# sstadick/gzp

Measured on AMD Instinct MI355X. Metric: BGZF compress MiB/s at level 1, 550 MiB text, higher is better.
Workload: dtype u8; 1 GPU; Single MI355X: 64 KiB BGZF blocks, level 1, 550 MiB text slab, bit-exact vs libdeflate; slab_bytes=576716800, block_size=65280, blocks=8835, level=1, format=bgzf, parallelism=block-shard x1, device=AMD Radeon Graphics (gfx950:sramecc+:xnack-, 256 CUs)

## Files before the change

### gzp_amd/csrc/gzpx_api.cpp

```cpp
#include <hip/hip_runtime.h>

#include <atomic>
#include <condition_variable>
#include <cmath>
#include <cstdio>
#include <cstdlib>
#include <mutex>
#include <new>
#include <string.h>
#include <vector>

#include "../../include/gzpx.h"
#include "gzpx_device.h"

using namespace gzpx;

namespace {

constexpr size_t kDictSize = 32768;
constexpr uint32_t kMaxBatchBlocks = 16384;
constexpr size_t kMaxScratchBytes = (size_t)24 << 30;

uint32_t multmodp(uint32_t a, uint32_t b) {
    uint32_t m = 1u << 31, p = 0;
// ... 305 lines not shown
                  uint8_t *d_out, size_t out_cap, hipStream_t stream, const SlabResult *prev,
                  SlabResult *result, hipEvent_t dom_b = nullptr, hipEvent_t dom_e = nullptr) {
    const Config &c = ctx->dcfg;
    const Scratch &s = ctx->scratch;
    ProfPairs pp{ctx, ctx->profiling != 0};
    pp.dom_b = dom_b;
    pp.dom_e = dom_e;
    ctx->prof_n = 0;
    auto fork_crc = [&]() -> int {
        HIP_TRY(hipEventRecord(ctx->ev_meta, stream));
        HIP_TRY(hipStreamWaitEvent(ctx->s_side, ctx->ev_meta, 0));
        pp.touch(stream);
        const int tc = pp.begin(6, ctx->s_side);
        launch_crc32(c, d_in, in_len, nb, s, ctx->crc_consts, ctx->s_side);
        pp.end(tc, ctx->s_side);
        HIP_TRY(hipEventRecord(ctx->ev_crc, ctx->s_side));
        return GZPX_OK;
    };
    const uint32_t fork_sel = (c.debug >> 8) & 3u;
    const uint32_t fork_at = fork_sel == 0 ? (c.level <= 1 ? 1u : 0u) : fork_sel == 1 ? 0u : fork_sel == 2 ? 2u : 1u;
    int t = pp.begin(c.level == 0 ? 0 : 1, stream);
    launch_candidates(c, d_in, in_len, nb, is_last, s, stream);
    pp.end(t, stream);
    if (fork_at == 1) {
        const int rc = fork_crc();
        if (rc != GZPX_OK) return rc;
    }
    if (c.level <= 1) {
        t = pp.begin(2, stream);
        launch_match(c, d_in, in_len, nb, s, stream);
        pp.end(t, stream);
        if (fork_at == 2) {
            const int rc = fork_crc();
            if (rc != GZPX_OK) return rc;
        }
        t = pp.begin(3, stream);
        launch_parse(c, d_in, in_len, nb, s, stream);
        pp.end(t, stream);
    } else {
        t = pp.begin(2, stream);
        if (c.level >= 10) {
            launch_near_optimal(c, d_in, nb, s, stream);
        } else if (c.lazy) {
            launch_lazy(c, d_in, nb, s, stream);
        } else {
            launch_hc(c, d_in, nb, s, stream);
        }
        pp.end(t, stream);
    }
    if (fork_at == 0 || (fork_at == 2 && c.level > 1)) {
        const int rc = fork_crc();
        if (rc != GZPX_OK) return rc;
    }
    t = pp.begin(4, stream);
    launch_hist(c, nb, s, stream);
    pp.end(t, stream);
    t = pp.begin(5, stream);
    launch_huffman(c, nb, s, stream);
    pp.end(t, stream);
    t = pp.begin(7, stream);
    launch_scan(nb, s, prev, result, stream);
    pp.end(t, stream);
    HIP_TRY(hipStreamWaitEvent(stream, ctx->ev_crc, 0));
    pp.touch(stream);
    t = pp.begin(8, stream);
    launch_emit(c, d_in, in_len, nb, s, d_out, out_cap, stream);
    pp.end(t, stream);
    HIP_TRY(hipGetLastError());
    if (pp.on && !dom_b) {
        HIP_TRY(hipStreamSynchronize(stream));
        for (int i = 0; i < ctx->prof_n; i++) {
            float ms = 0;
            HIP_TRY(hipEventElapsedTime(&ms, ctx->prof_ev[ctx->prof_b[i]], ctx->prof_ev[ctx->prof_e[i]]));
            ctx->stage_ms[ctx->prof_stage[i]] += ms;
        }
    }
    ctx->last_nb = nb;
    return GZPX_OK;
}

int enqueue_snap_batch(gzpx_ctx *ctx, const uint8_t *d_in, size_t in_len, uint32_t nb, uint8_t *d_out,
                       size_t out_cap, hipStream_t stream, const SlabResult *prev, SlabResult *result,
                       hipEvent_t dom_b = nullptr, hipEvent_t dom_e = nullptr) {
    const Scratch &s = ctx->scratch;
    const uint32_t bs = (uint32_t)ctx->cfg.buffer_size;
    ProfPairs pp{ctx, ctx->profiling != 0};
    pp.dom_b = dom_b;
    pp.dom_e = dom_e;
    ctx->prof_n = 0;
    if (ctx->snap.dbg)
        HIP_TRY(hipMemsetAsync(ctx->snap.dbg, 0,
                               (size_t)nb * snap_chunks_per_buffer(bs) * 8 * sizeof(uint64_t), stream));
    int t = pp.begin(2, stream);
    launch_snap_chunk(d_in, in_len, bs, nb, ctx->snap, stream);
    pp.end(t, stream);
    t = pp.begin(7, stream);
    launch_snap_frame(in_len, bs, nb, s, ctx->snap, stream);
    launch_scan(nb, s, prev, result, stream);
    pp.end(t, stream);
    t = pp.begin(8, stream);
    launch_snap_emit(d_in, in_len, bs, nb, s, ctx->snap, d_out, out_cap, stream);
    pp.end(t, stream);
    HIP_TRY(hipGetLastError());
    if (pp.on && !dom_b) {
        HIP_TRY(hipStreamSynchronize(stream));
        for (int i = 0; i < ctx->prof_n; i++) {
            float ms = 0;
            HIP_TRY(hipEventElapsedTime(&ms, ctx->prof_ev[ctx->prof_b[i]], ctx->prof_ev[ctx->prof_e[i]]));
            ctx->stage_ms[ctx->prof_stage[i]] += ms;
// ... 2121 lines not shown
```

### gzp_amd/csrc/gzpx_device.h

```cpp
#pragma once
#include <stdint.h>

namespace gzpx {

constexpr unsigned kTile = 65536;
constexpr unsigned kMaxBlockSize = 1u << 26;
constexpr unsigned kSeqPerSub = 8192;
constexpr unsigned kSoftMaxSub = 65535;
constexpr unsigned kMinBlockLen = 5000;
constexpr unsigned kNumLitlen = 288;
constexpr unsigned kNumOffset = 32;
constexpr unsigned kHistStride = kNumLitlen + kNumOffset;
constexpr unsigned kHdrWords = 160;
constexpr unsigned kCodeWords = kNumLitlen + kNumOffset;

constexpr uint32_t kTokMatch = 0x80000000u;

enum SubType : uint32_t { kStored = 0, kStatic = 1, kDynamic = 2 };

enum BlockStatus : uint32_t {
    kStatusOk = 0,
    kStatusBlockSizeExceeded = 2,
    kStatusInternal = 3,
};
// ... 69 lines not shown
    uint8_t *len8;
    uint32_t *which;
    uint16_t *alt;
    uint16_t *d4;
    uint8_t *lz_len;
    uint16_t *lz_dist;
    HcState *hc;
    uint32_t *pending;
    uint32_t *tok;
    uint32_t *redo;
    uint32_t *claim;
    uint32_t *hist;
    uint32_t *codes;
    uint32_t *hdr;
    uint64_t *out_off;
    uint32_t *sizes;
    uint32_t no_lanes;
    void *no_state;
    uint8_t *no_cache;
    uint8_t *no_nodes;
};

constexpr uint32_t kSnapStageBytes = 76544;
struct SnapScratch {
    uint8_t *stage;
    uint32_t *clen;
    uint32_t *crc;
    uint32_t *coff;
    uint64_t *dbg;
};
inline uint32_t snap_chunks_per_buffer(uint32_t bs) { return (bs + 65535u) / 65536u; }
void launch_snap_chunk(const uint8_t *slab, uint64_t slab_len, uint32_t bs, uint32_t nb, const SnapScratch &ss,
                       hipStream_t stream);
void launch_snap_frame(uint64_t slab_len, uint32_t bs, uint32_t nb, const Scratch &s, const SnapScratch &ss,
                       hipStream_t stream);
void launch_snap_emit(const uint8_t *slab, uint64_t slab_len, uint32_t bs, uint32_t nb, const Scratch &s,
                      const SnapScratch &ss, uint8_t *out, uint64_t out_cap, hipStream_t stream);

void launch_init_meta(const Config &cfg, uint64_t slab_len, uint32_t nb, int is_last,
                      const Scratch &s, hipStream_t stream);
void launch_candidates(const Config &cfg, const uint8_t *slab, uint64_t slab_len, uint32_t nb, int is_last,
                       const Scratch &s, hipStream_t stream);
void launch_match(const Config &cfg, const uint8_t *slab, uint64_t slab_len, uint32_t nb,
                  const Scratch &s, hipStream_t stream);
void launch_parse(const Config &cfg, const uint8_t *slab, uint64_t slab_len, uint32_t nb,
                  const Scratch &s, hipStream_t stream);
void launch_hc(const Config &cfg, const uint8_t *slab, uint32_t nb, const Scratch &s, hipStream_t stream);
void launch_lazy(const Config &cfg, const uint8_t *slab, uint32_t nb, const Scratch &s, hipStream_t stream);
size_t no_lane_bytes();
size_t no_cache_bytes();
size_t no_nodes_bytes(uint32_t block_size);
void launch_near_optimal_tables(void *lanes, uint32_t n_lanes, const uint8_t *d_tables, hipStream_t stream);
void launch_near_optimal(const Config &cfg, const uint8_t *slab, uint32_t nb, const Scratch &s, hipStream_t stream);
void launch_hist(const Config &cfg, uint32_t nb, const Scratch &s, hipStream_t stream);
void launch_huffman(const Config &cfg, uint32_t nb, const Scratch &s, hipStream_t stream);
void launch_crc32(const Config &cfg, const uint8_t *slab, uint64_t slab_len, uint32_t nb,
                  const Scratch &s, const CrcConsts &cc, hipStream_t stream);
void launch_scan(uint32_t nb, const Scratch &s, const SlabResult *prev, SlabResult *result, hipStream_t stream);
void launch_emit(const Config &cfg, const uint8_t *slab, uint64_t slab_len, uint32_t nb,
                 const Scratch &s, uint8_t *out, uint64_t out_cap, hipStream_t stream);

struct DBlockHost {
    uint64_t in_off;
    uint32_t size, isize, crc, status, produced, nmatch;
    uint32_t cyc[8];
};
struct InflateScratch {
    void *mlist = nullptr;
    uint32_t *tfirst = nullptr;
    uint32_t *redo = nullptr;
    uint32_t *summary = nullptr;
    int n_cu = 0;
    int big_members = 0;
};
enum { kInflateRouteSeg = 0, kInflateRouteWave = 1 };
size_t inflate_mlist_bytes(uint64_t out_cap, uint64_t nb);
size_t inflate_tfirst_bytes(uint64_t out_cap, uint64_t nb);
void launch_inflate(uint32_t hdr_len, const uint8_t *d_in, const uint64_t *d_offsets, const uint32_t *d_sizes,
                    uint32_t nb, void *d_blk, uint64_t *d_out_off, uint8_t *d_out, uint64_t out_cap,
                    uint32_t *d_crc_found, const CrcConsts &cc, int debug, hipEvent_t ev_begin,
                    hipEvent_t ev_end, hipStream_t stream, const InflateScratch &sc, int route, hipEvent_t ev_mid = nullptr);

struct MemberScanScratch {
    uint32_t *seg_count = nullptr;
    uint32_t *seg_off = nullptr;
    uint64_t *pos = nullptr;
    uint32_t *size = nullptr;
    uint32_t *succ = nullptr;
    uint32_t *jump[2] = {nullptr, nullptr};
    uint32_t *idx = nullptr;
    uint32_t *rec = nullptr;
    uint32_t cap = 0;
};
void launch_member_scan(int format, const uint8_t *d_in, uint64_t in_len, uint32_t seg_bytes, uint32_t n_seg,
                        uint32_t rounds, const MemberScanScratch &m, hipStream_t stream);
void launch_member_emit(const MemberScanScratch &m, uint32_t n_emit, uint64_t *d_offsets, uint32_t *d_sizes,
                        hipStream_t stream);
void launch_member_index(const uint8_t *d_in, const uint64_t *d_offsets, const uint32_t *d_sizes, uint32_t nb, void *d_blk,
                         uint64_t *d_out_off, hipStream_t stream);

struct RrIndex {
    const uint64_t *off;
    const uint32_t *size;
    const uint64_t *ustart;
    uint32_t n;
};
// ... 21 lines not shown
```

### gzp_amd/csrc/gzpx_kernels.hip

```cpp
#include <hip/hip_runtime.h>
#include <type_traits>
#include <cstring>

#include "gzpx_device.h"

#ifdef GZPX_EXPERIMENT
#define GZPX_EXP(cfg, bit) (((cfg).debug >> (bit)) & 1u)
#else
#define GZPX_EXP(cfg, bit) 0u
#endif

namespace gzpx {


__device__ __forceinline__ void wave_sync() {
    __builtin_amdgcn_fence(__ATOMIC_SEQ_CST, "wavefront");
    __builtin_amdgcn_wave_barrier();
    __builtin_amdgcn_fence(__ATOMIC_SEQ_CST, "wavefront");
}

__device__ __forceinline__ uint32_t rdlane(uint32_t v, uint32_t l) {
    return (uint32_t)__builtin_amdgcn_readlane((int)v, (int)l);
}
__device__ __forceinline__ uint32_t uniform(uint32_t v) { return (uint32_t)__builtin_amdgcn_readfirstlane((int)v); }

#if defined(__HIP_DEVICE_COMPILE__)
#define GZPX_PIN_VGPR(x) asm volatile("" : "+v"(x))
#else
#define GZPX_PIN_VGPR(x) ((void)0)
#endif

__device__ __forceinline__ uint32_t lz_hash15(uint32_t v) { return (v * 0x1E35A7BDu) >> 17; }

__device__ __forceinline__ uint32_t load_le32_global(const uint8_t *p) {
    const uintptr_t a = (uintptr_t)p;
    const uint32_t *w = (const uint32_t *)(a & ~(uintptr_t)3);
    return __builtin_amdgcn_alignbyte(w[1], w[0], (uint32_t)(a & 3));
}

__device__ __forceinline__ uint32_t wave_reduce_add(uint32_t v) {
    for (int m = 32; m >= 1; m >>= 1) v += __shfl_xor(v, m);
    return v;
}

__device__ __forceinline__ uint32_t wave_inclusive_scan(uint32_t v, unsigned lane) {
    for (int d = 1; d < 64; d <<= 1) {
        uint32_t t = __shfl_up(v, d);
        if (lane >= (unsigned)d) v += t;
    }
    return v;
}

template <int CTRL, int ROW_MASK>
__device__ __forceinline__ uint32_t dpp_zero(uint32_t v) {
// ... 2791 lines not shown
        }
        __syncthreads();
    }
}

struct HuffLds {
    union {
        uint32_t key[kNumLitlen];
        uint32_t nfreq[kNumLitlen];
        uint32_t hdr[kHdrWords];
    };
    union {
        uint32_t sfreq[kNumLitlen];
        struct {
            uint32_t sfreq_low[32];
            uint16_t items[kNumLitlen + kNumOffset];
        };
    };
    union {
        uint32_t freq[kNumLitlen];
        struct {
            uint32_t freq_low[kNumLitlen / 2];
            uint16_t parent[kNumLitlen];
        };
    };
    uint32_t lcw[kNumLitlen];
    uint16_t ssym[kNumLitlen];
    uint8_t depth[kNumLitlen];
    uint8_t lens[kNumLitlen + kNumOffset];
    uint8_t olens[kNumOffset + 2];
    uint8_t plens[32];
    uint32_t ocw[kNumOffset];
    uint32_t pcw[32];
    uint32_t pfreq[32];
    uint32_t len_counts[16];
    uint32_t misc[8];
};
static_assert(sizeof(HuffLds) <= 6400, "HuffLds: 25 workgroups per CU");
static_assert(kHdrWords <= kNumLitlen, "header bits fit region A");


__device__ __forceinline__ uint32_t reg5_get(const uint32_t (&r)[5], uint32_t k) {
    const uint32_t j = k >> 6, l = k & 63u;
    uint32_t v = rdlane(r[0], l);
    const uint32_t v1 = rdlane(r[1], l), v2 = rdlane(r[2], l), v3 = rdlane(r[3], l), v4 = rdlane(r[4], l);
    v = j == 1 ? v1 : v;
    v = j == 2 ? v2 : v;
    v = j == 3 ? v3 : v;
    v = j == 4 ? v4 : v;
    return v;
}

template <uint32_t NCH, uint32_t MAXL>
__device__ void make_code(HuffLds &h, uint32_t num_syms, uint32_t compat, uint8_t *lens, uint32_t *cw, uint32_t lane) {
    constexpr uint32_t max_len = MAXL;
    uint32_t used = 0;
    for (uint32_t base = 0; base < num_syms; base += 64) {
        const uint32_t s = base + lane;
        uint32_t f = 0;
        if (s < num_syms) {
            f = h.freq[s];
            h.key[s] = f ? ((f << 10) | s) : 0xFFFFFFFFu;
            lens[s] = 0;
            cw[s] = 0;
        }
        used += (uint32_t)__popcll(__ballot(f != 0));
    }
    wave_sync();
    if (used < 2) {
        if (used == 0 && compat == 1) return;
        if (lane == 0) {
            uint32_t sym = 0;
            if (used)
                for (uint32_t s = 0; s < num_syms; s++)
                    if (h.freq[s]) sym = s;
            const uint32_t other = sym ? sym : 1;
            lens[0] = 1;
            cw[0] = 0;
            lens[other] = 1;
            cw[other] = 1;
        }
        wave_sync();
        return;
    }
    {
        uint32_t at = 0;
        uint32_t k0 = lane < num_syms ? h.key[lane] : 0xFFFFFFFFu;
        for (uint32_t base = 0; base < num_syms; base += 64) {
            const uint32_t s1 = base + 64 + lane;
            const uint32_t k1 = s1 < num_syms ? h.key[s1] : 0xFFFFFFFFu;
            wave_sync();
            const bool u = k0 != 0xFFFFFFFFu;
            const unsigned long long m = __ballot(u);
            if (u) h.key[at + (uint32_t)__popcll(m & ((1ull << lane) - 1ull))] = k0;
            at += (uint32_t)__popcll(m);
            k0 = k1;
        }
    }
    wave_sync();
    for (uint32_t base = 0; base < used; base += 64) {
        const uint32_t s = base + lane;
        const uint32_t k = s < used ? h.key[s] : 0u;
        uint32_t rank = 0;
        for (uint32_t j = 0; j < used; j++) rank += h.key[j] < k ? 1u : 0u;
        if (s < used) {
            h.sfreq[rank] = k >> 10;
            h.ssym[rank] = (uint16_t)(k & 1023u);
// ... 82 lines not shown
                h.len_counts[l]--;
                h.len_counts[l + 1] += 2;
            }
        }
    }
    wave_sync();
    for (uint32_t base = 0; base < used; base += 64) {
        const uint32_t k = base + lane;
        if (k < used) {
            uint32_t acc = 0, l = max_len;
            for (; l >= 1; l--) {
                acc += h.len_counts[l];
                if (k < acc) break;
            }
            lens[h.ssym[k]] = (uint8_t)l;
        }
    }
    wave_sync();
    uint32_t next_code[16];
    next_code[0] = 0;
    next_code[1] = 0;
#pragma unroll
    for (uint32_t l = 2; l <= MAXL; l++) next_code[l] = (next_code[l - 1] + h.len_counts[l - 1]) << 1;
    const uint64_t lane_below = (1ull << lane) - 1ull;
    for (uint32_t base = 0; base < num_syms; base += 64) {
        const uint32_t s = base + lane;
        const uint32_t myl = s < num_syms ? lens[s] : 0;
        uint32_t code = 0;
#pragma unroll
        for (uint32_t l = 1; l <= MAXL; l++) {
            const uint64_t m = __ballot(myl == l);
            if (myl == l) code = next_code[l] + (uint32_t)__popcll(m & lane_below);
            next_code[l] += (uint32_t)__popcll(m);
        }
        if (myl) cw[s] = __brev(code) >> (32 - myl);
    }
    wave_sync();
}

__device__ __forceinline__ void hdr_or_bits(uint32_t *hdr, uint32_t bitpos, uint32_t v, uint32_t nbits) {
    const uint32_t w = bitpos >> 5, sh = bitpos & 31u;
    atomicOr(&hdr[w], v << sh);
    if (sh + nbits > 32) atomicOr(&hdr[w + 1], v >> (32 - sh));
}

__device__ __forceinline__ void hdr_put(uint32_t *hdr, uint32_t &bitpos, uint32_t v, uint32_t nbits) {
    if (!nbits) return;
    const uint32_t w = bitpos >> 5, sh = bitpos & 31u;
    hdr[w] |= v << sh;
    if (sh + nbits > 32) hdr[w + 1] |= v >> (32 - sh);
    bitpos += nbits;
}

#ifndef GZPX_HUFF_WAVES
#define GZPX_HUFF_WAVES 6
#endif
__global__ __launch_bounds__(64, GZPX_HUFF_WAVES) void k_huffman(Config cfg, BlockMeta *__restrict__ meta_all,
                                                SubMeta *__restrict__ sub_all,
                                                const uint32_t *__restrict__ hist_all,
                                                uint32_t *__restrict__ codes_all,
                                                uint32_t *__restrict__ hdr_all) {
    __shared__ HuffLds h;
    const uint32_t lane = threadIdx.x;
    const uint32_t b = blockIdx.x;
    BlockMeta *meta = meta_all + b;
    SubMeta *sub = sub_all + (uint64_t)b * cfg.max_sub;
    const uint32_t n = meta->n;
    const uint32_t hdr_len = hdr_len_of(cfg.format);
    const uint32_t eof_len = (meta->is_last && cfg.format == 0) ? 28u : 0u;

    if (n <= cfg.passthrough) {
        if (lane == 0) {
            const uint32_t chunks = n ? (n + 65534u) / 65535u : 1u;
            const uint32_t c = 5u * chunks + n;
            meta->nsub = 1;
            meta->ntok = 0;
            sub[0].type = kStored;
            sub[0].tok_begin = 0;
            sub[0].tok_end = 0;
            sub[0].byte_begin = 0;
            sub[0].byte_len = n;
            sub[0].bit_begin = 0;
            sub[0].hdr_bits = 0;
            sub[0].is_final = 1;
            meta->payload_bytes = c;
            meta->framed_bytes = hdr_len + c + 8 + eof_len;
            if (cfg.format == 0 && c >= 65536u) meta->status = kStatusBlockSizeExceeded;
        }
        return;
    }

    const uint32_t nsub = meta->nsub;
    uint32_t bitpos = 0;
    for (uint32_t s = 0; s < nsub; s++) {
        const uint32_t *hist = hist_all + ((uint64_t)b * cfg.max_sub + s) * kHistStride;
        uint32_t *codes = codes_all + ((uint64_t)b * cfg.max_sub + s) * kCodeWords;
        uint32_t *hdr_out = hdr_all + ((uint64_t)b * cfg.max_sub + s) * kHdrWords;
        const uint32_t block_length = sub[s].byte_len;
        const uint32_t is_final = sub[s].is_final;

#ifdef GZPX_EXPERIMENT
        unsigned long long hx_t = __builtin_readcyclecounter();
#define GZPX_HLAP(slot)                                                                               \
    do {                                                                                              \
        const unsigned long long t_ = __builtin_readcyclecounter();                                   \
        if (lane == 0) atomicAdd(&g_exp_huff[(b & 1023u) * 8u + (slot)], t_ - hx_t);                  \
        hx_t = t_;                                                                                    \
    } while (0)
#else
#define GZPX_HLAP(slot) ((void)0)
#endif
        uint32_t lfreq[5];
        for (uint32_t k = 0; k < 5; k++) {
            const uint32_t i = lane + 64 * k;
            lfreq[k] = i < kNumLitlen ? hist[i] + (i == 256 ? 1u : 0u) : 0;
            if (i < kNumLitlen) h.freq[i] = lfreq[k];
        }
        wave_sync();
        GZPX_HLAP(0);
        make_code<5, 14>(h, kNumLitlen, cfg.compat, h.lens, h.lcw, lane);
        GZPX_HLAP(1);
        const uint32_t ofreq = lane < kNumOffset ? hist[kNumLitlen + lane] : 0;
        if (lane < kNumOffset) h.freq[lane] = ofreq;
        wave_sync();
        make_code<1, 15>(h, kNumOffset, cfg.compat, h.olens, h.ocw, lane);
        GZPX_HLAP(2);
        wave_sync();

        uint32_t num_litlen, num_offset;
        {
            uint32_t hi_l = 0;
            for (uint32_t k = 0; k < 5; k++) {
                const uint32_t i = lane + 64 * k;
                if (i < kNumLitlen && h.lens[i]) hi_l = i + 1;
            }
            for (int m = 32; m >= 1; m >>= 1) {
                const uint32_t o = __shfl_xor(hi_l, m);
                hi_l = o > hi_l ? o : hi_l;
            }
            num_litlen = hi_l < 257 ? 257 : hi_l;
            uint32_t hi_o = (lane < kNumOffset && h.olens[lane]) ? lane + 1 : 0;
            for (int m = 32; m >= 1; m >>= 1) {
                const uint32_t o = __shfl_xor(hi_o, m);
                hi_o = o > hi_o ? o : hi_o;
            }
            num_offset = hi_o < 1 ? 1 : hi_o;
        }
        if (lane < num_offset) h.lens[num_litlen + lane] = h.olens[lane];
        if (lane < 32) h.pfreq[lane] = 0;
        wave_sync();
        uint32_t num_items;
        {
            const uint32_t num_lens = num_litlen + num_offset;
            uint32_t lr[5];
            unsigned long long sm[5];
#pragma unroll
            for (uint32_t k = 0; k < 5; k++) {
                const uint32_t idx = lane + 64 * k;
                lr[k] = idx < num_lens ? (uint32_t)h.lens[idx] : 0xFFu;
            }
#pragma unroll
            for (uint32_t k = 0; k < 5; k++) {
                uint32_t prev = (uint32_t)__shfl_up((int)lr[k], 1);
                const uint32_t carry = k ? rdlane(lr[k ? k - 1 : 0], 63) : 0x100u;
                if (lane == 0) prev = carry;
                sm[k] = __ballot(lr[k] != prev);
            }
            uint32_t ni = 0;
#pragma unroll
            for (uint32_t k = 0; k < 5; k++) {
                if (64 * k >= num_lens) break;
                uint32_t before = 0, after = num_lens;
#pragma unroll
                for (uint32_t j = 0; j < 5; j++)
                    if (j < k && sm[j]) before = 64 * j + 63u - (uint32_t)__clzll((long long)sm[j]);
// ... 413 lines not shown
    uint64_t inc = mine;
    for (int d = 1; d < 64; d <<= 1) {
        const uint64_t t = __shfl_up(inc, d);
        if (lane >= (unsigned)d) inc += t;
    }
    if (lane == 63) wsum[wave] = inc;
    __syncthreads();
    uint64_t run = prev ? prev->total : 0;
    uint64_t total = run;
    for (uint32_t w = 0; w < kScanThreads / 64; w++) {
        const uint64_t v = wsum[w];
        if (w < wave) run += v;
        total += v;
    }
    run += inc - mine;
#pragma unroll 8
    for (uint32_t i = i0; i < i1; i++) {
        const uint32_t v = meta[i].framed_bytes;
        sizes[i] = v;
        out_off[i] = run;
        run += v;
    }
    if (tid == 0) {
        const uint32_t f = fail_s;
        out_off[nb] = total;
        result->total = total;
        result->fail_block = f;
        result->fail_status = f != 0xFFFFFFFFu ? meta[f].status : kStatusOk;
    }
}

constexpr uint32_t kStageWords = 18432;

__device__ __forceinline__ void stage_or_bits(uint32_t *stage, uint32_t bitpos, uint64_t v) {
    const uint32_t w = bitpos >> 5, sh = bitpos & 31u;
    const uint64_t t = v << sh;
    const uint32_t x0 = (uint32_t)t, x1 = (uint32_t)(t >> 32);
    const uint32_t x2 = sh ? (uint32_t)(v >> (64 - sh)) : 0u;
    if (x0) atomicOr(&stage[w], x0);
    if (x1) atomicOr(&stage[w + 1], x1);
    if (x2) atomicOr(&stage[w + 2], x2);
}

__device__ __forceinline__ void stage_put_byte(uint32_t *stage, uint32_t byte_idx, uint32_t v) {
    atomicOr(&stage[byte_idx >> 2], (v & 0xFFu) << (8u * (byte_idx & 3u)));
}

constexpr uint32_t kEmitThreads = 1024;

__device__ __forceinline__ void stage_flush(const uint32_t *stage, uint8_t *dst_aligned,
                                            uint32_t win_base, uint32_t upto, uint32_t lead,
                                            uint32_t end_byte, uint32_t tid) {
    const uint32_t words = (upto - win_base + 3) >> 2;
    for (uint32_t w = tid; w < words; w += kEmitThreads) {
        const uint32_t v = stage[w];
        const uint32_t b0 = win_base + 4 * w;
        if (b0 >= lead && b0 + 4 <= end_byte && b0 + 4 <= upto) {
            *(uint32_t *)(dst_aligned + b0) = v;
        } else {
            for (uint32_t k = 0; k < 4; k++)
                if (b0 + k >= lead && b0 + k < end_byte && b0 + k < upto)
                    dst_aligned[b0 + k] = (uint8_t)(v >> (8 * k));
        }
    }
}

__device__ __forceinline__ void emit_block(const Config &cfg, const uint8_t *__restrict__ slab,
                                           const BlockMeta *__restrict__ meta_all,
                                           const SubMeta *__restrict__ sub_all,
                                           const uint32_t *__restrict__ tok_all,
                                           const uint32_t *__restrict__ codes_all,
                                           const uint32_t *__restrict__ hdr_all,
                                           const uint64_t *__restrict__ out_off,
                                           uint8_t *__restrict__ out, uint64_t out_cap, const uint32_t b,
                                           uint32_t *stage, uint32_t *codes, uint32_t *wsum, const uint8_t *lslot) {
    const uint32_t tid = threadIdx.x;
    const BlockMeta *meta = meta_all + b;
    const SubMeta *sub = sub_all + (uint64_t)b * cfg.max_sub;
    const uint32_t n = meta->n;
    const uint32_t framed = meta->framed_bytes;
    const uint32_t c = meta->payload_bytes;
    const uint64_t dst_off = out_off[b];
    if (meta->status != kStatusOk || dst_off + framed > out_cap) return;
    const uint8_t *in = slab + (uint64_t)b * cfg.block_size;
    const uint32_t hdr_len = hdr_len_of(cfg.format);
    const uint32_t lead = (uint32_t)(((uintptr_t)out + dst_off) & 3u);
    uint8_t *dst_aligned = out + dst_off - lead;
    const uint32_t end_byte = lead + framed;
    uint32_t win_base = 0;

    for (uint32_t i = tid; i < kStageWords; i += kEmitThreads) stage[i] = 0;
    __syncthreads();

    if (tid == 0) {
        const uint32_t hb = lead;
        stage_put_byte(stage, hb + 0, 0x1f);
        stage_put_byte(stage, hb + 1, 0x8b);
        stage_put_byte(stage, hb + 2, 8);
        stage_put_byte(stage, hb + 3, 4);
        stage_put_byte(stage, hb + 8, cfg.xfl);
        stage_put_byte(stage, hb + 9, 255);
        if (cfg.format == 0) {
            const uint32_t bsize = c + 25;
            stage_put_byte(stage, hb + 10, 6);
            stage_put_byte(stage, hb + 12, 'B');
            stage_put_byte(stage, hb + 13, 'C');
            stage_put_byte(stage, hb + 14, 2);
            stage_put_byte(stage, hb + 16, bsize);
            stage_put_byte(stage, hb + 17, bsize >> 8);
        } else {
            const uint32_t tot = c + 28;
            stage_put_byte(stage, hb + 10, 8);
            stage_put_byte(stage, hb + 12, 'I');
            stage_put_byte(stage, hb + 13, 'G');
            stage_put_byte(stage, hb + 14, 4);
            stage_put_byte(stage, hb + 16, tot);
            stage_put_byte(stage, hb + 17, tot >> 8);
            stage_put_byte(stage, hb + 18, tot >> 16);
            stage_put_byte(stage, hb + 19, tot >> 24);
        }
    }

    const uint32_t *tok = tok_all + (uint64_t)b * cfg.stride;
    const uint32_t nsub = meta->nsub;
    uint32_t bitpos = 8u * (lead + hdr_len);
    auto ensure = [&](uint32_t need_bits) {
        if (((bitpos + need_bits + 7) >> 3) + 16u <= 4u * kStageWords) return;
        __syncthreads();
        const uint32_t upto_rel = (bitpos >> 3) & ~3u;
        stage_flush(stage, dst_aligned, win_base, win_base + upto_rel, lead, end_byte, tid);
        const uint32_t keep = stage[upto_rel >> 2];
        __syncthreads();
        for (uint32_t i = tid; i < kStageWords; i += kEmitThreads) stage[i] = 0;
        __syncthreads();
        if (tid == 0) stage[0] = keep;
        win_base += upto_rel;
        bitpos -= 8u * upto_rel;
        __syncthreads();
    };
    for (uint32_t s = 0; s < nsub; s++) {
        const SubMeta sm = sub[s];
        if (sm.type == kStored) {
            uint32_t left = sm.byte_len, src = sm.byte_begin;
            do {
                const uint32_t chunk = left > 65535u ? 65535u : left;
                const bool last_chunk = chunk == left;
                ensure(64);
                if (tid == 0) stage_or_bits(stage, bitpos, (sm.is_final && last_chunk) ? 1u : 0u);
                bitpos = (bitpos + 3 + 7u) & ~7u;
                if (tid == 0) {
                    const uint32_t bytepos = bitpos >> 3;
                    stage_put_byte(stage, bytepos + 0, chunk);
                    stage_put_byte(stage, bytepos + 1, chunk >> 8);
                    stage_put_byte(stage, bytepos + 2, ~chunk);
                    stage_put_byte(stage, bytepos + 3, (~chunk) >> 8);
                }
                bitpos += 32;
                for (uint32_t done = 0; done < chunk; done += 16384u) {
                    const uint32_t piece = chunk - done < 16384u ? chunk - done : 16384u;
                    ensure(8u * piece);
                    const uint32_t bytepos = bitpos >> 3;
                    for (uint32_t i = tid; i < piece; i += kEmitThreads)
                        stage_put_byte(stage, bytepos + i, in[src + done + i]);
                    bitpos += 8u * piece;
                }
                src += chunk;
                left -= chunk;
            } while (left);
            __syncthreads();
            continue;
        }
        __syncthreads();
        const uint32_t *cd = codes_all + ((uint64_t)b * cfg.max_sub + s) * kCodeWords;
        for (uint32_t i = tid; i < kCodeWords; i += kEmitThreads) codes[i] = cd[i];
        const uint32_t *hw = hdr_all + ((uint64_t)b * cfg.max_sub + s) * kHdrWords;
        const uint32_t nhw = (sm.hdr_bits + 31) >> 5;
        ensure(32u * kHdrWords);
        for (uint32_t i = tid; i < nhw; i += kEmitThreads) stage_or_bits(stage, bitpos + 32 * i, hw[i]);
        bitpos += sm.hdr_bits;
        __syncthreads();
        const uint32_t tok_last = meta->ntok - 1;
        uint32_t tnext[4];
#pragma unroll
        for (uint32_t j = 0; j < 4; j++) {
            const uint32_t i = sm.tok_begin + 4 * tid + j;
            tnext[j] = tok[i < tok_last ? i : tok_last];
        }
        for (uint32_t tb = sm.tok_begin; tb < sm.tok_end; tb += 4 * kEmitThreads) {
            ensure(4u * kEmitThreads * 48u);
            const uint32_t t0 = tb + 4 * tid;
            uint64_t bits[4];
            uint32_t nbits[4], sum = 0;
            uint32_t tcur[4];
#pragma unroll
            for (uint32_t j = 0; j < 4; j++) tcur[j] = tnext[j];
#pragma unroll
            for (uint32_t j = 0; j < 4; j++) {
                const uint32_t i = t0 + 4 * kEmitThreads + j;
                tnext[j] = tok[i < tok_last ? i : tok_last];
            }
#pragma unroll
            for (uint32_t j = 0; j < 4; j++) {
                bits[j] = 0;
                nbits[j] = 0;
                if (t0 + j < sm.tok_end) {
                    const uint32_t t = tcur[j];
                    if (t & kTokMatch) {
                        const uint32_t len = t & 0x1FFu, off = (t >> 9) & 0xFFFFu;
                        uint32_t os, oe, ov;
                        const uint32_t lt = lslot[len - 3u];
                        const uint32_t ls = lt & 31u, le = lt >> 5, lv = (len - 3u) & ((1u << le) - 1u);
                        offset_slot(off, os, oe, ov);
                        const uint32_t lc = codes[257 + ls], oc = codes[kNumLitlen + os];
                        const uint32_t lpart = (lc & 0xFFFFu) | (lv << (lc >> 16)), lbits = (lc >> 16) + le;
                        const uint32_t opart = (oc & 0xFFFFu) | (ov << (oc >> 16)), obits = (oc >> 16) + oe;
                        bits[j] = (uint64_t)lpart | ((uint64_t)opart << lbits);
                        nbits[j] = lbits + obits;
                    } else {
                        const uint32_t lc = codes[t];
                        bits[j] = lc & 0xFFFFu;
                        nbits[j] = lc >> 16;
                    }
                    sum += nbits[j];
                }
            }
            uint32_t total;
            const uint32_t ex = block_exclusive_scan<kEmitThreads / 64>(sum, wsum, &total);
            uint32_t off_bits = bitpos + ex, accn = 0;
            uint64_t acc = 0;
#pragma unroll
            for (uint32_t j = 0; j < 4; j++) {
                if (accn + nbits[j] > 64) {
                    stage_or_bits(stage, off_bits, acc);
                    off_bits += accn;
                    acc = 0;
                    accn = 0;
                }
                acc |= bits[j] << accn;
                accn += nbits[j];
            }
            if (accn) stage_or_bits(stage, off_bits, acc);
            bitpos += total;
        }
        ensure(64);
        if (tid == 0) {
            const uint32_t ec = codes[256];
            stage_or_bits(stage, bitpos, ec & 0xFFFFu);
        }
        bitpos += codes[256] >> 16;
        __syncthreads();
    }

    ensure(8u * (8u + 28u + 8u));
    if (tid == 0) {
        const uint32_t fb = lead + hdr_len + c - win_base;
        const uint32_t crc = meta->crc;
        for (uint32_t k = 0; k < 4; k++) {
            stage_put_byte(stage, fb + k, crc >> (8 * k));
            stage_put_byte(stage, fb + 4 + k, n >> (8 * k));
        }
        if (meta->is_last && cfg.format == 0) {
            const uint8_t eof[28] = {0x1f, 0x8b, 0x08, 0x04, 0, 0, 0, 0, 0x00, 0xff, 0x06, 0x00, 0x42, 0x43,
                                     0x02, 0x00, 0x1b, 0x00, 0x03, 0x00, 0, 0, 0, 0, 0, 0, 0, 0};
            for (uint32_t k = 0; k < 28; k++) stage_put_byte(stage, fb + 8 + k, eof[k]);
        }
    }
    __syncthreads();
    stage_flush(stage, dst_aligned, win_base, end_byte, lead, end_byte, tid);
}

__global__ __launch_bounds__(kEmitThreads, 8) void k_emit(Config cfg, const uint8_t *__restrict__ slab,
                                              const BlockMeta *__restrict__ meta_all,
                                              const SubMeta *__restrict__ sub_all,
                                              const uint32_t *__restrict__ tok_all,
                                              const uint32_t *__restrict__ codes_all,
                                              const uint32_t *__restrict__ hdr_all,
                                              const uint64_t *__restrict__ out_off,
                                              uint8_t *__restrict__ out, uint64_t out_cap, uint32_t nb) {
    __shared__ uint32_t stage[kStageWords];
    __shared__ uint32_t codes[kCodeWords];
    __shared__ uint32_t wsum[kEmitThreads / 64];
    __shared__ uint8_t lslot[256];
    if (threadIdx.x < 256) {
        uint32_t ls, le, lv;
        length_slot(threadIdx.x + 3, ls, le, lv);
        lslot[threadIdx.x] = (uint8_t)(ls | (le << 5));
    }
    for (uint32_t b = blockIdx.x; b < nb; b += gridDim.x) {
        __syncthreads();
        emit_block(cfg, slab, meta_all, sub_all, tok_all, codes_all, hdr_all, out_off, out, out_cap, b, stage, codes, wsum,
                   lslot);
    }
}

template <bool GWIN>
struct InfLdsT {
    uint32_t win[GWIN ? 1 : 8192];
    uint32_t lfast[1024];
    uint32_t ofast[256];
    uint32_t inr[256];
    uint32_t own[64];
    uint16_t lsorted[288];
    uint16_t osorted[32];
    uint8_t lens[320];
    uint32_t lcount[16], lfirst[16], loffs[16];
    uint32_t ocount[16], ofirst[16], ooffs[16];
};

#ifndef GZPX_INF_R
#define GZPX_INF_R 2
#endif
constexpr uint32_t kInfR = GZPX_INF_R;

enum InflateStatus : uint32_t { kInfOk = 0, kInfBadData = 1, kInfInsufficientSpace = 2, kInfShortOutput = 3 };

enum InfKind { kInfLitlen = 0, kInfOffset = 1, kInfPrecode = 2 };

template <int KIND>
__device__ __forceinline__ uint32_t inflate_entry(uint32_t sym, uint32_t cl) {
    if (KIND == kInfPrecode) return cl | (sym << 8);
    if (KIND == kInfLitlen) {
        if (sym < 256) return cl | (sym << 8);
        if (sym == 256) return cl | (2u << 4);
        const uint32_t slot = sym - 257;
        uint32_t base, xb = 0;
        if (slot < 8) {
            base = 3 + slot;
        } else if (slot >= 28) {
            base = 258;
        } else {
            xb = (slot - 4) >> 2;
            base = 3 + ((4 + (slot & 3)) << xb);
        }
        return cl | (1u << 4) | (xb << 8) | (base << 16);
    }
    if (sym > 29) return cl | (1u << 4);
    uint32_t base, xb = 0;
    if (sym < 4) {
        base = 1 + sym;
    } else {
        xb = (sym - 2) >> 1;
        base = 1 + ((2 + (sym & 1)) << xb);
    }
    return cl | (xb << 8) | (base << 16);
// ... 838 lines not shown
        hipLaunchKernelGGL(k_match_hc, dim3(nb), dim3(1024), 0, stream, cfg, slab, (const BlockMeta *)s.meta, s.hc,
                           (const uint16_t *)s.cand, (const uint16_t *)s.d4, s.len8, s.which, s.alt,
                           (uint8_t *)nullptr, (uint16_t *)nullptr);
    };
    auto parse_round = [&](uint32_t may_list_stale) {
        hipLaunchKernelGGL(k_parse_hc<false>, dim3(nb), dim3(kMpThreads), 0, stream, cfg, slab, s.meta, s.sub, s.hc,
                           (const uint8_t *)s.len8, (const uint32_t *)s.which, (const uint16_t *)s.alt, s.tok,
                           s.pending, s.redo, may_list_stale);
    };
    const bool sparse = !(cfg.debug & 16u) && (cfg.level >= 3 || (cfg.debug & 32u));
    if (sparse)
        hipLaunchKernelGGL(k_match_hc_sparse, dim3(nb), dim3(1024), 0, stream, cfg, slab, (const BlockMeta *)s.meta, s.hc,
                           (const uint16_t *)s.cand, (const uint16_t *)s.d4, s.len8, s.which, s.alt);
    else
        dense();
    hipLaunchKernelGGL(k_hc_orphan, dim3(nb), dim3(64), 0, stream, cfg, slab, (const BlockMeta *)s.meta, s.hc,
                       (const uint16_t *)s.cand, (const uint16_t *)s.d4, s.len8, s.which, s.alt, (uint8_t *)nullptr,
                       (uint16_t *)nullptr);
    parse_round(1u);
    if (sparse) {
        const uint32_t wgs = cfg.n_cu ? cfg.n_cu : 256u;
        hipLaunchKernelGGL(k_match_hc_stale, dim3(wgs), dim3(1024), 0, stream, cfg, slab, (const BlockMeta *)s.meta,
                           s.hc, (const uint16_t *)s.cand, (const uint16_t *)s.d4, s.len8, s.which, s.alt,
                           (const uint32_t *)s.redo);
    }
    parse_round(0u);
    hipLaunchKernelGGL(k_parse_hc<true>, dim3(nb), dim3(kMpThreads), 0, stream, cfg, slab, s.meta, s.sub, s.hc,
                       (const uint8_t *)s.len8, (const uint32_t *)s.which, (const uint16_t *)s.alt, s.tok,
                       s.pending, s.redo, 0u);
}

void launch_lazy(const Config &cfg, const uint8_t *slab, uint32_t nb, const Scratch &s, hipStream_t stream) {
    hipLaunchKernelGGL(k_hc_init, dim3((nb + 255) / 256), dim3(256), 0, stream, nb, s.hc, s.pending);
    hipLaunchKernelGGL(k_match_hc, dim3(nb), dim3(1024), 0, stream, cfg, slab, (const BlockMeta *)s.meta, s.hc,
                       (const uint16_t *)s.cand, (const uint16_t *)s.d4, s.len8, s.which, s.alt, s.lz_len,
                       s.lz_dist);
    hipLaunchKernelGGL(k_hc_orphan, dim3(nb), dim3(64), 0, stream, cfg, slab, (const BlockMeta *)s.meta, s.hc,
                       (const uint16_t *)s.cand, (const uint16_t *)s.d4, s.len8, s.which, s.alt, s.lz_len, s.lz_dist);
    if (cfg.lazy >= 2)
        hipLaunchKernelGGL(k_parse_lazy<3>, dim3(nb), dim3(64), 0, stream, cfg, slab, s.meta, s.sub,
                           (const uint8_t *)s.len8, (const uint16_t *)s.alt, (const uint8_t *)s.lz_len,
                           (const uint16_t *)s.lz_dist, s.tok);
    else
        hipLaunchKernelGGL(k_parse_lazy<2>, dim3(nb), dim3(64), 0, stream, cfg, slab, s.meta, s.sub,
                           (const uint8_t *)s.len8, (const uint16_t *)s.alt, (const uint8_t *)s.lz_len,
                           (const uint16_t *)s.lz_dist, s.tok);
}

void launch_hist(const Config &cfg, uint32_t nb, const Scratch &s, hipStream_t stream) {
    hipLaunchKernelGGL(k_hist, dim3(nb), dim3(256), 0, stream, cfg, (const BlockMeta *)s.meta,
                       (const SubMeta *)s.sub, (const uint32_t *)s.tok, s.hist);
}

void launch_huffman(const Config &cfg, uint32_t nb, const Scratch &s, hipStream_t stream) {
    hipLaunchKernelGGL(k_huffman, dim3(nb), dim3(64), 0, stream, cfg, s.meta, s.sub,
                       (const uint32_t *)s.hist, s.codes, s.hdr);
}

void launch_crc32(const Config &cfg, const uint8_t *slab, uint64_t, uint32_t nb, const Scratch &s,
                  const CrcConsts &cc, hipStream_t stream) {
    hipLaunchKernelGGL(k_crc32, dim3(nb), dim3(kCrcSmall), 0, stream, cfg, slab, s.meta, cc);
}

void launch_scan(uint32_t nb, const Scratch &s, const SlabResult *prev, SlabResult *result, hipStream_t stream) {
    hipLaunchKernelGGL(k_scan, dim3(1), dim3(kScanThreads), 0, stream, nb, (const BlockMeta *)s.meta,
                       s.out_off, s.sizes, prev, result);
}

void launch_emit(const Config &cfg, const uint8_t *slab, uint64_t, uint32_t nb, const Scratch &s,
                 uint8_t *out, uint64_t out_cap, hipStream_t stream) {
    hipLaunchKernelGGL(k_emit, dim3(nb), dim3(kEmitThreads), 0, stream, cfg, slab, (const BlockMeta *)s.meta,
                       (const SubMeta *)s.sub, (const uint32_t *)s.tok, (const uint32_t *)s.codes,
                       (const uint32_t *)s.hdr, (const uint64_t *)s.out_off, out, out_cap, nb);
}

void launch_inflate(uint32_t hdr_len, const uint8_t *d_in, const uint64_t *d_offsets, const uint32_t *d_sizes,
                    uint32_t nb, void *d_blk, uint64_t *d_out_off, uint8_t *d_out, uint64_t out_cap,
                    uint32_t *d_crc_found, const CrcConsts &cc, int debug, hipEvent_t ev_begin,
                    hipEvent_t ev_end, hipStream_t stream, const InflateScratch &sc, int route, hipEvent_t ev_mid) {
    DBlock *blk = (DBlock *)d_blk;
    const bool seg = route != kInflateRouteWave && sc.mlist && sc.tfirst && sc.redo;
    hipLaunchKernelGGL(k_dinit, dim3((nb + 255) / 256), dim3(256), 0, stream, nb, d_in, d_offsets, d_sizes, blk,
                       seg ? sc.redo : (uint32_t *)nullptr);
    hipLaunchKernelGGL(k_dscan, dim3(1), dim3(256), 0, stream, nb, (const DBlock *)blk, d_out_off);
    if (ev_begin) (void)hipEventRecord(ev_begin, stream);
    if (seg) {
        LzMatch *ml = (LzMatch *)sc.mlist;
        const bool big = sc.big_members != 0;
        const uint32_t seg_wgs = (uint32_t)(sc.n_cu > 0 ? sc.n_cu : 256) * 4u * GZPX_SEG_WAVES / (big ? (uint32_t)kSegBigW : (uint32_t)kSegSmallW);
        const uint32_t seg_grid = nb < seg_wgs ? nb : seg_wgs;
        uint32_t *seg_hint = sc.summary ? sc.summary + 15 : nullptr;
#define GZPX_LAUNCH_SEG(DBG_)                                                                                              \
    do {                                                                                                                   \
        if (big)                                                                                                           \
            hipLaunchKernelGGL((k_inflate_seg<DBG_, kSegBigW>), dim3(seg_grid), dim3(64 * kSegBigW), 0, stream, hdr_len,   \
                               d_in, blk, (const uint64_t *)d_out_off, d_out, out_cap, ml, sc.tfirst, sc.redo, nb, seg_hint); \
        else                                                                                                               \
            hipLaunchKernelGGL((k_inflate_seg<DBG_, kSegSmallW>), dim3(seg_grid), dim3(64 * kSegSmallW), 0, stream, hdr_len, d_in, blk, \
                               (const uint64_t *)d_out_off, d_out, out_cap, ml, sc.tfirst, sc.redo, nb, seg_hint);         \
        if (ev_mid) (void)hipEventRecord(ev_mid, stream);                                                                  \
    } while (0)
        if (debug == 1) {
            GZPX_LAUNCH_SEG(true);
            hipLaunchKernelGGL((k_lzcopy<false>), dim3(nb), dim3(kLcThreads), 0, stream, blk, (const uint64_t *)d_out_off,
                               d_out, (const LzMatch *)ml, (const uint32_t *)sc.tfirst, sc.redo, d_crc_found, cc);
            hipLaunchKernelGGL((k_inflate<true, true>), dim3(nb), dim3(64), 0, stream, hdr_len, d_in, blk,
                               (const uint64_t *)d_out_off, d_out, out_cap, (const uint32_t *)sc.redo);
        } else if (debug == 2) {
            GZPX_LAUNCH_SEG(false);
// ... 91 lines not shown
```

Baseline: 159,700 MiB/s.

## Fold symbol histogram into the Huffman kernel and skip separate hist launch

When the block size fits in one tile, the Huffman kernel now tallies literal/length and offset frequencies itself from the token stream. It uses LDS atomics over four padded copies and a length-slot lookup table, so the separate histogram kernel launch and its global hist buffer round trip are dropped. The tally runs with a single 64-lane wave per block instead of the 256-thread hist kernel, which trades launch and global-memory traffic for a longer serial phase inside the Huffman kernel. The tally lives in a union overlaid on the existing LDS struct, so occupancy is meant to stay the same.

```diff
diff --git a/gzp_amd/csrc/gzpx_api.cpp b/gzp_amd/csrc/gzpx_api.cpp
--- a/gzp_amd/csrc/gzpx_api.cpp
+++ b/gzp_amd/csrc/gzpx_api.cpp
@@ -381,9 +381,11 @@
         const int rc = fork_crc();
         if (rc != GZPX_OK) return rc;
     }
-    t = pp.begin(4, stream);
-    launch_hist(c, nb, s, stream);
-    pp.end(t, stream);
+    if (!huffman_tallies(c)) {
+        t = pp.begin(4, stream);
+        launch_hist(c, nb, s, stream);
+        pp.end(t, stream);
+    }
     t = pp.begin(5, stream);
     launch_huffman(c, nb, s, stream);
     pp.end(t, stream);
diff --git a/gzp_amd/csrc/gzpx_device.h b/gzp_amd/csrc/gzpx_device.h
--- a/gzp_amd/csrc/gzpx_device.h
+++ b/gzp_amd/csrc/gzpx_device.h
@@ -145,6 +145,7 @@
 size_t no_nodes_bytes(uint32_t block_size);
 void launch_near_optimal_tables(void *lanes, uint32_t n_lanes, const uint8_t *d_tables, hipStream_t stream);
 void launch_near_optimal(const Config &cfg, const uint8_t *slab, uint32_t nb, const Scratch &s, hipStream_t stream);
+bool huffman_tallies(const Config &cfg);
 void launch_hist(const Config &cfg, uint32_t nb, const Scratch &s, hipStream_t stream);
 void launch_huffman(const Config &cfg, uint32_t nb, const Scratch &s, hipStream_t stream);
 void launch_crc32(const Config &cfg, const uint8_t *slab, uint64_t slab_len, uint32_t nb,
diff --git a/gzp_amd/csrc/gzpx_kernels.hip b/gzp_amd/csrc/gzpx_kernels.hip
--- a/gzp_amd/csrc/gzpx_kernels.hip
+++ b/gzp_amd/csrc/gzpx_kernels.hip
@@ -1,5 +1,6 @@
 #include <hip/hip_runtime.h>
 #include <type_traits>
+#include <cstddef>
 #include <cstring>
 
 #include "gzpx_device.h"
@@ -2897,7 +2898,7 @@
 }
 
 template <uint32_t NCH, uint32_t MAXL>
-__device__ void make_code(HuffLds &h, uint32_t num_syms, uint32_t compat, uint8_t *lens, uint32_t *cw, uint32_t lane) {
+__device__ __forceinline__ void make_code(HuffLds &h, uint32_t num_syms, uint32_t compat, uint8_t *lens, uint32_t *cw, uint32_t lane) {
     constexpr uint32_t max_len = MAXL;
     uint32_t used = 0;
     for (uint32_t base = 0; base < num_syms; base += 64) {
@@ -3086,15 +3087,75 @@
     bitpos += nbits;
 }
 
+constexpr uint32_t kTallyCopies = 4;
+constexpr uint32_t kTallyLitPad = kNumLitlen + 1;
+constexpr uint32_t kTallyOffPad = kNumOffset + 1;
+constexpr uint32_t kTallyOffAt = kTallyCopies * kTallyLitPad;
+constexpr uint32_t kTallyWords = kTallyOffAt + kTallyCopies * kTallyOffPad;
+union HuffShared {
+    HuffLds h;
+    struct {
+        uint32_t tally[kTallyWords];
+        uint8_t lslot[512];
+    };
+};
+static_assert(sizeof(HuffShared) == sizeof(HuffLds), "the tally lives inside HuffLds: 24 workgroups per CU as before");
+static_assert(kTallyWords * 4 + 512 <= offsetof(HuffLds, ocw), "the tally ends in front of ocw[]");
+
+template <bool EDGE>
+__device__ __forceinline__ void huff_tally_token(uint32_t t, bool in, uint32_t *lit, uint32_t *off, const uint8_t *lslot) {
+    const bool m = (t & kTokMatch) != 0;
+    const uint32_t ls = lslot[t & 0x1FFu];
+    if (!EDGE || in) atomicAdd(&lit[m ? 257u + ls : t], 1u);
+    if ((!EDGE || in) && m) {
+        const uint32_t d = ((t >> 9) & 0xFFFFu) - 1u;
+        const uint32_t ko = 30u - (uint32_t)__clz((int)(d | 2u));
+        atomicAdd(&off[(ko << 1) + (d >> ko)], 1u);
+    }
+}
+
+__device__ __forceinline__ void huff_tally(HuffShared &sh, const uint32_t *__restrict__ tok, uint32_t t_begin,
+                                           uint32_t t_end, uint32_t lane) {
+    constexpr uint32_t U = 4;
+    uint32_t *lit = sh.tally + (lane & (kTallyCopies - 1u)) * kTallyLitPad;
+    uint32_t *off = sh.tally + kTallyOffAt + (lane & (kTallyCopies - 1u)) * kTallyOffPad;
+    for (uint32_t base = t_begin & ~3u; base < t_end; base += 4u * 64u * U) {
+        const uint32_t q0 = base + 4u * lane;
+        uint4 v[U];
+#pragma unroll
+        for (uint32_t k = 0; k < U; k++) {
+            const uint32_t q = q0 + 4u * 64u * k;
+            v[k] = q < t_end ? *reinterpret_cast<const uint4 *>(tok + q) : make_uint4(~0u, ~0u, ~0u, ~0u);
+        }
+        const bool inside = base >= t_begin && base + 4u * 64u * U <= t_end;
+#pragma unroll
+        for (uint32_t k = 0; k < U; k++) {
+            const uint32_t q = q0 + 4u * 64u * k;
+            const uint32_t e4[4] = {v[k].x, v[k].y, v[k].z, v[k].w};
+            if (inside) {
+#pragma unroll
+                for (uint32_t e = 0; e < 4; e++) huff_tally_token<false>(e4[e], true, lit, off, sh.lslot);
+            } else {
+#pragma unroll
+                for (uint32_t e = 0; e < 4; e++)
+                    huff_tally_token<true>(e4[e], q + e - t_begin < t_end - t_begin, lit, off, sh.lslot);
+            }
+        }
+    }
+}
+
 #ifndef GZPX_HUFF_WAVES
 #define GZPX_HUFF_WAVES 6
 #endif
+template <bool TALLY>
 __global__ __launch_bounds__(64, GZPX_HUFF_WAVES) void k_huffman(Config cfg, BlockMeta *__restrict__ meta_all,
                                                 SubMeta *__restrict__ sub_all,
                                                 const uint32_t *__restrict__ hist_all,
+                                                const uint32_t *__restrict__ tok_all,
                                                 uint32_t *__restrict__ codes_all,
                                                 uint32_t *__restrict__ hdr_all) {
-    __shared__ HuffLds h;
+    __shared__ HuffShared sh;
+    HuffLds &h = sh.h;
     const uint32_t lane = threadIdx.x;
     const uint32_t b = blockIdx.x;
     BlockMeta *meta = meta_all + b;
@@ -3125,6 +3186,7 @@
     }
 
     const uint32_t nsub = meta->nsub;
+    const uint32_t *tok = tok_all + (uint64_t)b * cfg.stride;
     uint32_t bitpos = 0;
     for (uint32_t s = 0; s < nsub; s++) {
         const uint32_t *hist = hist_all + ((uint64_t)b * cfg.max_sub + s) * kHistStride;
@@ -3145,16 +3207,48 @@
 #define GZPX_HLAP(slot) ((void)0)
 #endif
         uint32_t lfreq[5];
+        uint32_t ofreq = 0;
+        if (TALLY) {
+            for (uint32_t i = lane; i < kTallyWords; i += 64) sh.tally[i] = 0;
+            for (uint32_t i = lane; i < 512; i += 64) {
+                uint32_t ls = 0, le, lv;
+                if (i >= 3 && i <= 258) length_slot(i, ls, le, lv);
+                sh.lslot[i] = (uint8_t)ls;
+            }
+            wave_sync();
+            huff_tally(sh, tok, sub[s].tok_begin, sub[s].tok_end, lane);
+            wave_sync();
+#pragma unroll
+            for (uint32_t k = 0; k < 5; k++) {
+                const uint32_t i = lane + 64 * k;
+                uint32_t f = i == 256 ? 1u : 0u;
+                if (i < kNumLitlen) {
+#pragma unroll
+                    for (uint32_t c = 0; c < kTallyCopies; c++) f += sh.tally[c * kTallyLitPad + i];
+                }
+                lfreq[k] = f;
+            }
+            if (lane < kNumOffset) {
+#pragma unroll
+                for (uint32_t c = 0; c < kTallyCopies; c++) ofreq += sh.tally[kTallyOffAt + c * kTallyOffPad + lane];
+                h.ocw[lane] = ofreq;
+            }
+            wave_sync();
+        } else {
+            for (uint32_t k = 0; k < 5; k++) {
+                const uint32_t i = lane + 64 * k;
+                lfreq[k] = i < kNumLitlen ? hist[i] + (i == 256 ? 1u : 0u) : 0;
+            }
+        }
         for (uint32_t k = 0; k < 5; k++) {
             const uint32_t i = lane + 64 * k;
-            lfreq[k] = i < kNumLitlen ? hist[i] + (i == 256 ? 1u : 0u) : 0;
             if (i < kNumLitlen) h.freq[i] = lfreq[k];
         }
         wave_sync();
         GZPX_HLAP(0);
         make_code<5, 14>(h, kNumLitlen, cfg.compat, h.lens, h.lcw, lane);
         GZPX_HLAP(1);
-        const uint32_t ofreq = lane < kNumOffset ? hist[kNumLitlen + lane] : 0;
+        ofreq = lane < kNumOffset ? (TALLY ? h.ocw[lane] : hist[kNumLitlen + lane]) : 0;
         if (lane < kNumOffset) h.freq[lane] = ofreq;
         wave_sync();
         make_code<1, 15>(h, kNumOffset, cfg.compat, h.olens, h.ocw, lane);
@@ -4856,9 +4950,15 @@
                        (const SubMeta *)s.sub, (const uint32_t *)s.tok, s.hist);
 }
 
+bool huffman_tallies(const Config &cfg) { return cfg.block_size <= kTile && !(cfg.debug & 128u); }
+
 void launch_huffman(const Config &cfg, uint32_t nb, const Scratch &s, hipStream_t stream) {
-    hipLaunchKernelGGL(k_huffman, dim3(nb), dim3(64), 0, stream, cfg, s.meta, s.sub,
-                       (const uint32_t *)s.hist, s.codes, s.hdr);
+    if (huffman_tallies(cfg))
+        hipLaunchKernelGGL(k_huffman<true>, dim3(nb), dim3(64), 0, stream, cfg, s.meta, s.sub, (const uint32_t *)s.hist,
+                           (const uint32_t *)s.tok, s.codes, s.hdr);
+    else
+        hipLaunchKernelGGL(k_huffman<false>, dim3(nb), dim3(64), 0, stream, cfg, s.meta, s.sub, (const uint32_t *)s.hist,
+                           (const uint32_t *)s.tok, s.codes, s.hdr);
 }
 
 void launch_crc32(const Config &cfg, const uint8_t *slab, uint64_t, uint32_t nb, const Scratch &s,
```

After: 160,900 MiB/s, median of 6. No clear change (+0.8%).

## Precompute per-subblock literal/length code table and branchless token emission in k_emit

Applied to the files above, without the earlier changes.

Builds a 512-entry LDS table per sub-block holding literal codes and length codes with their extra bits already merged, and replaces the per-token branch with a branchless path that reads this table and derives the offset slot with clz. When no pair of tokens in a wave exceeds 64 bits, it writes two paired 64-bit ORs instead of the general accumulator loop. It also zeroes only the part of the stage buffer the block actually uses, with 16-byte stores, and makes the flush loop unconditional word stores with only the edge words handled bytewise. The costs are an extra table build per sub-block and a wave-uniform any() vote.

```diff
diff --git a/gzp_amd/csrc/gzpx_kernels.hip b/gzp_amd/csrc/gzpx_kernels.hip
--- a/gzp_amd/csrc/gzpx_kernels.hip
+++ b/gzp_amd/csrc/gzpx_kernels.hip
@@ -3674,17 +3674,42 @@
                                             uint32_t win_base, uint32_t upto, uint32_t lead,
                                             uint32_t end_byte, uint32_t tid) {
     const uint32_t words = (upto - win_base + 3) >> 2;
-    for (uint32_t w = tid; w < words; w += kEmitThreads) {
-        const uint32_t v = stage[w];
-        const uint32_t b0 = win_base + 4 * w;
-        if (b0 >= lead && b0 + 4 <= end_byte && b0 + 4 <= upto) {
-            *(uint32_t *)(dst_aligned + b0) = v;
-        } else {
+    const uint32_t lim = upto < end_byte ? upto : end_byte;
+    const uint32_t lo_b = win_base > lead ? win_base : (lead + 3u) & ~3u;
+    const uint32_t w_lo = (lo_b - win_base) >> 2;
+    const uint32_t w_hi = lim > lo_b ? w_lo + ((lim - lo_b) >> 2) : w_lo;
+    for (uint32_t w = w_lo + tid; w < w_hi; w += kEmitThreads) *(uint32_t *)(dst_aligned + win_base + 4 * w) = stage[w];
+    if (tid < 2) {
+        const uint32_t w = tid ? w_hi : w_lo - 1u;
+        if (w < words && (tid || w_lo)) {
+            const uint32_t v = stage[w];
+            const uint32_t b0 = win_base + 4 * w;
             for (uint32_t k = 0; k < 4; k++)
-                if (b0 + k >= lead && b0 + k < end_byte && b0 + k < upto)
-                    dst_aligned[b0 + k] = (uint8_t)(v >> (8 * k));
-        }
-    }
+                if (b0 + k >= lead && b0 + k < lim) dst_aligned[b0 + k] = (uint8_t)(v >> (8 * k));
+        }
+    }
+}
+
+struct TokenReads {
+    uint32_t lt, oc, d, e;
+};
+
+__device__ __forceinline__ TokenReads token_reads(uint32_t t, const uint32_t *ltab, const uint32_t *codes) {
+    TokenReads r;
+    r.lt = ltab[(t & 0x1FFu) + ((uint32_t)((int32_t)t >> 31) & 253u)];
+    r.d = ((t - 512u) >> 9) & 0xFFFFu;
+    r.e = 30u - (uint32_t)__clz((int)(r.d | 2u));
+    r.oc = codes[kNumLitlen + (r.d >> r.e) + 2u * r.e];
+    return r;
+}
+
+__device__ __forceinline__ uint64_t token_bits(uint32_t t, const TokenReads &r, uint32_t &n) {
+    const uint32_t m = (uint32_t)((int32_t)t >> 31);
+    const uint32_t lpart = r.lt & 0xFFFFFu, lbits = r.lt >> 20;
+    const uint32_t ov = r.d & ((1u << r.e) - 1u);
+    const uint32_t opart = ((r.oc & 0xFFFFu) | (ov << (r.oc >> 16))) & m, obits = ((r.oc >> 16) + r.e) & m;
+    n = lbits + obits;
+    return (uint64_t)lpart | ((uint64_t)opart << lbits);
 }
 
 __device__ __forceinline__ void emit_block(const Config &cfg, const uint8_t *__restrict__ slab,
@@ -3695,7 +3720,7 @@
                                            const uint32_t *__restrict__ hdr_all,
                                            const uint64_t *__restrict__ out_off,
                                            uint8_t *__restrict__ out, uint64_t out_cap, const uint32_t b,
-                                           uint32_t *stage, uint32_t *codes, uint32_t *wsum, const uint8_t *lslot) {
+                                           uint32_t *stage, uint32_t *codes, uint32_t *wsum, uint32_t *ltab) {
     const uint32_t tid = threadIdx.x;
     const BlockMeta *meta = meta_all + b;
     const SubMeta *sub = sub_all + (uint64_t)b * cfg.max_sub;
@@ -3711,7 +3736,11 @@
     const uint32_t end_byte = lead + framed;
     uint32_t win_base = 0;
 
-    for (uint32_t i = tid; i < kStageWords; i += kEmitThreads) stage[i] = 0;
+    {
+        const uint32_t zw = (end_byte + 3u) / 4u + 3u;
+        const uint32_t zq = zw < kStageWords ? (zw + 3u) / 4u : kStageWords / 4u;
+        for (uint32_t i = tid; i < zq; i += kEmitThreads) ((uint4 *)stage)[i] = make_uint4(0u, 0u, 0u, 0u);
+    }
     __syncthreads();
 
     if (tid == 0) {
@@ -3795,6 +3824,21 @@
         __syncthreads();
         const uint32_t *cd = codes_all + ((uint64_t)b * cfg.max_sub + s) * kCodeWords;
         for (uint32_t i = tid; i < kCodeWords; i += kEmitThreads) codes[i] = cd[i];
+        if (tid < 512) {
+            uint32_t part, nb;
+            if (tid < 256) {
+                const uint32_t lc = cd[tid];
+                part = lc & 0xFFFFu;
+                nb = lc >> 16;
+            } else {
+                uint32_t ls, le, lv;
+                length_slot(tid - 256u + 3u, ls, le, lv);
+                const uint32_t lc = cd[257 + ls];
+                part = (lc & 0xFFFFu) | (lv << (lc >> 16));
+                nb = (lc >> 16) + le;
+            }
+            ltab[tid] = part | (nb << 20);
+        }
         const uint32_t *hw = hdr_all + ((uint64_t)b * cfg.max_sub + s) * kHdrWords;
         const uint32_t nhw = (sm.hdr_bits + 31) >> 5;
         ensure(32u * kHdrWords);
@@ -3821,47 +3865,64 @@
                 const uint32_t i = t0 + 4 * kEmitThreads + j;
                 tnext[j] = tok[i < tok_last ? i : tok_last];
             }
-#pragma unroll
-            for (uint32_t j = 0; j < 4; j++) {
-                bits[j] = 0;
-                nbits[j] = 0;
-                if (t0 + j < sm.tok_end) {
-                    const uint32_t t = tcur[j];
-                    if (t & kTokMatch) {
-                        const uint32_t len = t & 0x1FFu, off = (t >> 9) & 0xFFFFu;
-                        uint32_t os, oe, ov;
-                        const uint32_t lt = lslot[len - 3u];
-                        const uint32_t ls = lt & 31u, le = lt >> 5, lv = (len - 3u) & ((1u << le) - 1u);
-                        offset_slot(off, os, oe, ov);
-                        const uint32_t lc = codes[257 + ls], oc = codes[kNumLitlen + os];
-                        const uint32_t lpart = (lc & 0xFFFFu) | (lv << (lc >> 16)), lbits = (lc >> 16) + le;
-                        const uint32_t opart = (oc & 0xFFFFu) | (ov << (oc >> 16)), obits = (oc >> 16) + oe;
-                        bits[j] = (uint64_t)lpart | ((uint64_t)opart << lbits);
-                        nbits[j] = lbits + obits;
-                    } else {
-                        const uint32_t lc = codes[t];
-                        bits[j] = lc & 0xFFFFu;
-                        nbits[j] = lc >> 16;
+            const uint32_t wave_t0 = __builtin_amdgcn_readfirstlane(tb + 4 * (tid & ~63u));
+            bool paired = wave_t0 + 256u <= sm.tok_end;
+            if (paired) {
+                TokenReads rd[4];
+#pragma unroll
+                for (uint32_t j = 0; j < 4; j++) rd[j] = token_reads(tcur[j], ltab, codes);
+#pragma unroll
+                for (uint32_t j = 0; j < 4; j++) bits[j] = token_bits(tcur[j], rd[j], nbits[j]);
+                paired = !__any(nbits[0] + nbits[1] > 64u || nbits[2] + nbits[3] > 64u);
+                sum = (nbits[0] + nbits[1]) + (nbits[2] + nbits[3]);
+            } else {
+#pragma unroll
+                for (uint32_t j = 0; j < 4; j++) {
+                    bits[j] = 0;
+                    nbits[j] = 0;
+                    if (t0 + j < sm.tok_end) {
+                        const uint32_t t = tcur[j];
+                        if (t & kTokMatch) {
+                            const uint32_t len = t & 0x1FFu, off = (t >> 9) & 0xFFFFu;
+                            uint32_t os, oe, ov;
+                            const uint32_t lt = ltab[256u + len - 3u];
+                            offset_slot(off, os, oe, ov);
+                            const uint32_t oc = codes[kNumLitlen + os];
+                            const uint32_t lpart = lt & 0xFFFFFu, lbits = lt >> 20;
+                            const uint32_t opart = (oc & 0xFFFFu) | (ov << (oc >> 16)), obits = (oc >> 16) + oe;
+                            bits[j] = (uint64_t)lpart | ((uint64_t)opart << lbits);
+                            nbits[j] = lbits + obits;
+                        } else {
+                            const uint32_t lc = codes[t];
+                            bits[j] = lc & 0xFFFFu;
+                            nbits[j] = lc >> 16;
+                        }
+                        sum += nbits[j];
                     }
-                    sum += nbits[j];
                 }
             }
             uint32_t total;
             const uint32_t ex = block_exclusive_scan<kEmitThreads / 64>(sum, wsum, &total);
             uint32_t off_bits = bitpos + ex, accn = 0;
-            uint64_t acc = 0;
-#pragma unroll
-            for (uint32_t j = 0; j < 4; j++) {
-                if (accn + nbits[j] > 64) {
-                    stage_or_bits(stage, off_bits, acc);
-                    off_bits += accn;
-                    acc = 0;
-                    accn = 0;
-                }
-                acc |= bits[j] << accn;
-                accn += nbits[j];
-            }
-            if (accn) stage_or_bits(stage, off_bits, acc);
+            if (paired) {
+                const uint32_t n01 = nbits[0] + nbits[1];
+                stage_or_bits(stage, off_bits, bits[0] | (bits[1] << nbits[0]));
+                stage_or_bits(stage, off_bits + n01, bits[2] | (bits[3] << nbits[2]));
+            } else {
+                uint64_t acc = 0;
+#pragma unroll
+                for (uint32_t j = 0; j < 4; j++) {
+                    if (accn + nbits[j] > 64) {
+                        stage_or_bits(stage, off_bits, acc);
+                        off_bits += accn;
+                        acc = 0;
+                        accn = 0;
+                    }
+                    acc |= bits[j] << accn;
+                    accn += nbits[j];
+                }
+                if (accn) stage_or_bits(stage, off_bits, acc);
+            }
             bitpos += total;
         }
         ensure(64);
@@ -3899,19 +3960,14 @@
                                               const uint32_t *__restrict__ hdr_all,
                                               const uint64_t *__restrict__ out_off,
                                               uint8_t *__restrict__ out, uint64_t out_cap, uint32_t nb) {
-    __shared__ uint32_t stage[kStageWords];
+    __shared__ __attribute__((aligned(16))) uint32_t stage[kStageWords];
     __shared__ uint32_t codes[kCodeWords];
     __shared__ uint32_t wsum[kEmitThreads / 64];
-    __shared__ uint8_t lslot[256];
-    if (threadIdx.x < 256) {
-        uint32_t ls, le, lv;
-        length_slot(threadIdx.x + 3, ls, le, lv);
-        lslot[threadIdx.x] = (uint8_t)(ls | (le << 5));
-    }
+    __shared__ uint32_t ltab[512];
     for (uint32_t b = blockIdx.x; b < nb; b += gridDim.x) {
         __syncthreads();
         emit_block(cfg, slab, meta_all, sub_all, tok_all, codes_all, hdr_all, out_off, out, out_cap, b, stage, codes, wsum,
-                   lslot);
+                   ltab);
     }
 }
 
```

New measurement: 159,700 MiB/s before, 160,100 MiB/s after, median of 6. No clear change (+0.2%).
